# MoFHeka/MeepoEmbedding

Hardware: AMD Instinct MI355X
Metric: key-lookups/sec (higher is better)
Workload: dtype int64 keys / fp32 rows (copy)

## Files before the change

include/meepo_embedding.h:

```cpp
#ifndef MEEPO_EMBEDDING_H
#define MEEPO_EMBEDDING_H
#include <stddef.h>
#include <stdint.h>

#ifdef __cplusplus
extern "C" {
#endif

#define MEE_ABI_VERSION 2

#define MEE_EMPTY_KEY     INT64_MIN
#define MEE_RECLAIMED_KEY (INT64_MIN + 1)
#define MEE_BUCKET_WIDTH  16

enum { MEE_OK = 0, MEE_ERR_INVALID_ARG = -1, MEE_ERR_OUT_OF_MEMORY = -2, MEE_ERR_HIP = -3,
       MEE_ERR_NO_DEVICE = -4, MEE_ERR_BATCH_TOO_LARGE = -5, MEE_ERR_UNSUPPORTED = -6,
       MEE_ERR_RCCL = -7  };

enum { MEE_OPT_NONE = 0, MEE_OPT_ADAGRAD = 1, MEE_OPT_ADAM = 2 };
enum { MEE_INIT_CONSTANT = 0, MEE_INIT_UNIFORM = 1 };
enum { MEE_STATUS_TABLE_FULL = 1u, MEE_STATUS_RESERVED_KEY = 2u, MEE_STATUS_STALE_HANDLE = 4u, MEE_STATUS_INTERNAL = 8u };
enum { MEE_MEM_HBM = 0, MEE_MEM_HOST_PINNED = 1 };
enum { MEE_FLAG_TRACK_HITS = 1u, MEE_FLAG_ADMISSION = 2u };

// ... 175 lines not shown
                    void* stream);

int mee_bag_runs(mee_router* r, const int64_t* d_perm, const uint64_t* d_counts, size_t n, const uint64_t* d_bag_offsets, size_t n_bags,
                 uint32_t* d_run_bag, uint32_t* d_run_len, uint64_t* d_run_counts, void* stream);
int mee_run_offsets(mee_router* r, const uint32_t* d_run_len, size_t n_runs, uint64_t* d_offsets, uint32_t* d_run_of_key, size_t n_keys,
                    void* stream);
int mee_combine_bag_runs(mee_router* r, const float* d_partials, const uint32_t* d_run_bag, const uint64_t* d_run_counts, size_t n_runs,
                         const uint64_t* d_bag_offsets, size_t n_bags, uint32_t dim, int mode, void* d_out, uint32_t out_dtype, void* stream);

int mee_segment_counts(mee_router* r, const int64_t* d_perm, const uint64_t* d_counts, size_t n, const uint64_t* d_offsets, size_t n_tables,
                       uint64_t* d_cell_counts, void* stream);
int mee_regroup(mee_router* r, const int64_t* d_recv_keys, const uint64_t* d_recv_cells, size_t n_recv, size_t n_tables, int64_t* d_keys_out,
                int64_t* d_order_out, uint64_t* d_offsets_out, void* stream);

int mee_p2p_create(int32_t device, uint32_t n_shards, uint32_t rank, uint64_t slots_per_peer, uint64_t max_batch, uint32_t dim,
                   int with_payload, mee_p2p** out);
int mee_p2p_destroy(mee_p2p* c);
#define MEE_P2P_BUFFERS 6
int mee_p2p_export(mee_p2p* c, void* handles );
int mee_p2p_connect(mee_p2p* c, const void* all_handles );
int mee_p2p_buffers(mee_p2p* c, float** d_out, uint8_t** d_found);
int mee_p2p_push(mee_p2p* c, mee_router* r, const int64_t* d_send_keys, const int64_t* d_perm, const uint64_t* d_counts, size_t n,
                 void* stream);
int mee_p2p_find(mee_p2p* c, const mee_table* t, void* stream);
int mee_p2p_push_rows(mee_p2p* c, mee_router* r, const int64_t* d_send_keys, const int64_t* d_perm, const uint64_t* d_counts,
                      const float* d_rows, size_t n, void* stream);
int mee_p2p_inbox(mee_p2p* c, int64_t** d_keys, float** d_rows, uint64_t* n_slots);
int mee_p2p_barrier(mee_p2p* c, void* stream);
int mee_p2p_status(mee_p2p* c, uint32_t* bits_out, void* stream);


#define MEE_COMM_ID_BYTES 128
int mee_comm_unique_id(void* id_out );
int mee_comm_create(const void* id, uint32_t n_ranks, uint32_t rank, int32_t device, void** comm_out);
int mee_comm_destroy(void* comm);
int mee_comm_aborted(void* comm);
int mee_sharded_create(mee_table* local, void* nccl_comm, uint64_t max_batch ,
                       double pad_slack, mee_sharded** out);
enum { MEE_SHARDED_DEDUP = 1u };
typedef struct mee_sharded_options {
    uint32_t struct_size;
    uint32_t flags;
    uint64_t max_batch;
    double   pad_slack;
    mee_table* cold;
    uint64_t hot_key_limit;
} mee_sharded_options;
int mee_sharded_create_ex(mee_table* local, void* nccl_comm, const mee_sharded_options* options, mee_sharded** out);
int mee_sharded_destroy(mee_sharded* s);
int mee_sharded_info(const mee_sharded* s, uint32_t* n_shards, uint32_t* rank, uint64_t* segment_capacity );
int mee_sharded_find(mee_sharded* s, const int64_t* d_keys, size_t n, float* d_out, uint8_t* d_found , void* stream);
int mee_sharded_find_or_insert(mee_sharded* s, const int64_t* d_keys, size_t n, float* d_out, uint8_t* d_found, void* stream);
// ... 18 lines not shown
```

include/meepo_embedding.hpp:

```cpp
#pragma once
#include <cstdint>
#include <stdexcept>
#include <string>
#include <utility>

#include "meepo_embedding.h"

namespace meepo {

class Error : public std::runtime_error {
public:
    Error(int code, const std::string& msg) : std::runtime_error("meepo error " + std::to_string(code) + ": " + msg), code_(code) {}
    int code() const noexcept { return code_; }
private:
    int code_;
};

inline void check(int rc) {
    if (rc != MEE_OK) throw Error(rc, mee_last_error());
}

struct TableOptions {
    int32_t device = 0;
    uint64_t capacity = 0;
// ... 152 lines not shown
    Router(Router&& o) noexcept : r_(std::exchange(o.r_, nullptr)) {}
    Router(const Router&) = delete;
    Router& operator=(const Router&) = delete;
    mee_router* handle() const noexcept { return r_; }
    void partition(const int64_t* d_keys, size_t n, int64_t* d_send_keys, uint64_t* d_counts, int64_t* d_perm, void* stream = nullptr) { check(mee_partition(r_, d_keys, n, d_send_keys, d_counts, d_perm, stream)); }
    void partition_padded(const int64_t* d_keys, size_t n, int64_t* d_send_keys, uint64_t* d_counts, int64_t* d_perm, void* stream = nullptr) { check(mee_partition_padded(r_, d_keys, n, d_send_keys, d_counts, d_perm, stream)); }
    static void scatter_rows(const void* d_rows, const int64_t* d_perm, size_t n, size_t row_bytes, void* d_out, void* stream = nullptr) { check(mee_scatter_rows(d_rows, d_perm, n, row_bytes, d_out, stream)); }
    static void gather_rows(const void* d_rows, const int64_t* d_perm, size_t n, size_t row_bytes, void* d_out, void* stream = nullptr) { check(mee_gather_rows(d_rows, d_perm, n, row_bytes, d_out, stream)); }
private:
    mee_router* r_ = nullptr;
};

class PeerExchange {
public:
    PeerExchange(int32_t device, uint32_t n_shards, uint32_t rank, uint64_t slots_per_peer, uint64_t max_batch, uint32_t dim, bool with_payload = false) {
        check(mee_p2p_create(device, n_shards, rank, slots_per_peer, max_batch, dim, with_payload ? 1 : 0, &c_));
    }
    ~PeerExchange() { if (c_) mee_p2p_destroy(c_); }
    PeerExchange(const PeerExchange&) = delete;
    PeerExchange& operator=(const PeerExchange&) = delete;
    void export_handles(void* handles_6x64) { check(mee_p2p_export(c_, handles_6x64)); }
    void connect(const void* all_handles_rank_major) { check(mee_p2p_connect(c_, all_handles_rank_major)); }
    void push(Router& r, const int64_t* d_send_keys, const int64_t* d_perm, const uint64_t* d_counts, size_t n, void* stream = nullptr) { check(mee_p2p_push(c_, r.handle(), d_send_keys, d_perm, d_counts, n, stream)); }
    void find(const Table& t, void* stream = nullptr) { check(mee_p2p_find(c_, t.handle(), stream)); }
    void barrier(void* stream = nullptr) { check(mee_p2p_barrier(c_, stream)); }
    void push_rows(Router& r, const int64_t* d_send_keys, const int64_t* d_perm, const uint64_t* d_counts, const float* d_rows, size_t n, void* stream = nullptr) {
        check(mee_p2p_push_rows(c_, r.handle(), d_send_keys, d_perm, d_counts, d_rows, n, stream));
    }
    int64_t* inbox_keys() const { int64_t* k = nullptr; check(mee_p2p_inbox(c_, &k, nullptr, nullptr)); return k; }
    float* inbox_rows() const { float* r = nullptr; check(mee_p2p_inbox(c_, nullptr, &r, nullptr)); return r; }
    uint64_t inbox_slots() const { uint64_t n = 0; check(mee_p2p_inbox(c_, nullptr, nullptr, &n)); return n; }
    float* rows() const { float* o = nullptr; check(mee_p2p_buffers(c_, &o, nullptr)); return o; }
    uint8_t* found() const { uint8_t* f = nullptr; check(mee_p2p_buffers(c_, nullptr, &f)); return f; }
    uint32_t status(void* stream = nullptr) { uint32_t b = 0; check(mee_p2p_status(c_, &b, stream)); return b; }
private:
    mee_p2p* c_ = nullptr;
};

class Communicator {
public:
    static void unique_id(void* id_128_bytes) { check(mee_comm_unique_id(id_128_bytes)); }
    Communicator(const void* id_128_bytes, uint32_t n_ranks, uint32_t rank, int32_t device) { check(mee_comm_create(id_128_bytes, n_ranks, rank, device, &c_)); }
    ~Communicator() { if (c_) mee_comm_destroy(c_); }
    Communicator(const Communicator&) = delete;
    Communicator& operator=(const Communicator&) = delete;
    void* handle() const noexcept { return c_; }
private:
    void* c_ = nullptr;
};

class ShardedTable {
public:
    ShardedTable(Table& local, void* nccl_comm, uint64_t max_batch, double pad_slack = 0.0) { check(mee_sharded_create(local.handle(), nccl_comm, max_batch, pad_slack, &s_)); }
    ShardedTable(Table& local, void* nccl_comm, uint64_t max_batch, double pad_slack, Table* cold, uint32_t flags = 0, uint64_t hot_key_limit = 0) {
        mee_sharded_options o{};
        o.struct_size = sizeof o; o.flags = flags; o.max_batch = max_batch; o.pad_slack = pad_slack; o.cold = cold ? cold->handle() : nullptr; o.hot_key_limit = hot_key_limit;
        check(mee_sharded_create_ex(local.handle(), nccl_comm, &o, &s_));
// ... 23 lines not shown
```

meepoembedding_amd/_lib.py:

```python
from __future__ import annotations

import ctypes as C
import os

import torch

_HERE = os.path.dirname(os.path.abspath(__file__))
LIB_PATH = os.environ.get("MEE_LIB_PATH") or os.path.join(_HERE, "libmeepo_hip.so")

OK = 0
ERR_INVALID_ARG, ERR_OUT_OF_MEMORY, ERR_HIP, ERR_NO_DEVICE, ERR_BATCH_TOO_LARGE, ERR_UNSUPPORTED, ERR_RCCL = -1, -2, -3, -4, -5, -6, -7
OPT_NONE, OPT_ADAGRAD, OPT_ADAM = 0, 1, 2
INIT_CONSTANT, INIT_UNIFORM = 0, 1
STATUS_TABLE_FULL, STATUS_RESERVED_KEY, STATUS_STALE_HANDLE, STATUS_INTERNAL = 1, 2, 4, 8
FIND_DEFAULT, FIND_STREAM_STORES, FIND_CACHED_STORES, FIND_STREAM_ROWS, FIND_STREAM_BUCKETS = 0, 1, 2, 4, 8
HANDLE_SLOT_MASK = (1 << 40) - 1
MEM_HBM, MEM_HOST_PINNED = 0, 1
DTYPE_F32, DTYPE_BF16 = 0, 1
FLAG_TRACK_HITS, FLAG_ADMISSION = 1, 2
ABI_VERSION = 2
EMPTY_KEY = -(1 << 63)
RECLAIMED_KEY = EMPTY_KEY + 1
BUCKET_WIDTH = 16

# ... 108 lines not shown
    "mee_table_plane": (C.c_int, [_vp, _u32, C.POINTER(_vp), C.POINTER(_u64), C.POINTER(_u32)]),
    "mee_device_calibration": (C.c_int, [C.c_int32, C.POINTER(Calibration)]),
    "mee_probe_length": (C.c_int, [_vp, _vp, _sz, C.POINTER(_u64), _vp]),
    "mee_probe_histogram": (C.c_int, [_vp, _vp, _sz, C.POINTER(C.c_uint64), _vp]),
    "mee_apply_adagrad": (C.c_int, [_vp, _vp, _vp, _sz, _f32, _f32, _vp]),
    "mee_apply_adam": (C.c_int, [_vp, _vp, _vp, _sz, _f32, _f32, _f32, _f32, _u64, _vp]),
    "mee_apply_prepare": (C.c_int, [_vp, _vp, _sz, _vp]),
    "mee_apply_discard": (C.c_int, [_vp, _vp]),
    "mee_dedup_sum": (C.c_int, [_vp, _vp, _vp, _sz, _vp, _vp, _vp, _vp, C.c_int64, _vp]),
    "mee_hash_batch": (C.c_int, [_vp, _sz, _u64, _u32, _vp, _vp, _vp, _vp]),
    "mee_router_create": (C.c_int, [_i32, _u64, _u32, C.POINTER(_vp)]),
    "mee_router_destroy": (C.c_int, [_vp]),
    "mee_partition_padded": (C.c_int, [_vp, _vp, _sz, _vp, _vp, _vp, _vp]),
    "mee_partition": (C.c_int, [_vp, _vp, _sz, _vp, _vp, _vp, _vp]),
    "mee_p2p_create": (C.c_int, [_i32, _u32, _u32, _u64, _u64, _u32, C.c_int, C.POINTER(_vp)]),
    "mee_p2p_barrier": (C.c_int, [_vp, _vp]),
    "mee_p2p_push_rows": (C.c_int, [_vp, _vp, _vp, _vp, _vp, _vp, _sz, _vp]),
    "mee_p2p_inbox": (C.c_int, [_vp, C.POINTER(_vp), C.POINTER(_vp), C.POINTER(_u64)]),
    "mee_p2p_destroy": (C.c_int, [_vp]),
    "mee_p2p_export": (C.c_int, [_vp, _vp]),
    "mee_p2p_connect": (C.c_int, [_vp, _vp]),
    "mee_p2p_buffers": (C.c_int, [_vp, C.POINTER(_vp), C.POINTER(_vp)]),
    "mee_p2p_push": (C.c_int, [_vp, _vp, _vp, _vp, _vp, _sz, _vp]),
    "mee_p2p_find": (C.c_int, [_vp, _vp, _vp]),
    "mee_p2p_status": (C.c_int, [_vp, C.POINTER(_u32), _vp]),
    "mee_scatter_rows": (C.c_int, [_vp, _vp, _sz, _sz, _vp, _vp]),
    "mee_gather_rows": (C.c_int, [_vp, _vp, _sz, _sz, _vp, _vp]),
    "mee_bag_runs": (C.c_int, [_vp, _vp, _vp, _sz, _vp, _sz, _vp, _vp, _vp, _vp]),
    "mee_run_offsets": (C.c_int, [_vp, _vp, _sz, _vp, _vp, _sz, _vp]),
    "mee_combine_bag_runs": (C.c_int, [_vp, _vp, _vp, _vp, _sz, _vp, _sz, _u32, C.c_int, _vp, _u32, _vp]),
    "mee_segment_counts": (C.c_int, [_vp, _vp, _vp, _sz, _vp, _sz, _vp, _vp]),
    "mee_regroup": (C.c_int, [_vp, _vp, _vp, _sz, _sz, _vp, _vp, _vp, _vp]),
    "mee_comm_unique_id": (C.c_int, [_vp]),
    "mee_comm_create": (C.c_int, [_vp, _u32, _u32, _i32, C.POINTER(_vp)]),
    "mee_comm_destroy": (C.c_int, [_vp]),
    "mee_comm_aborted": (C.c_int, [_vp]),
    "mee_sharded_create": (C.c_int, [_vp, _vp, _u64, C.c_double, C.POINTER(_vp)]),
    "mee_sharded_create_ex": (C.c_int, [_vp, _vp, C.POINTER(ShardedOptions), C.POINTER(_vp)]),
    "mee_sharded_clear_status": (C.c_int, [_vp, _vp]),
    "mee_sharded_destroy": (C.c_int, [_vp]),
    "mee_sharded_info": (C.c_int, [_vp, C.POINTER(_u32), C.POINTER(_u32), C.POINTER(_u64)]),
    "mee_sharded_find": (C.c_int, [_vp, _vp, _sz, _vp, _vp, _vp]),
    "mee_sharded_find_or_insert": (C.c_int, [_vp, _vp, _sz, _vp, _vp, _vp]),
    "mee_sharded_find_as": (C.c_int, [_vp, _vp, _sz, _vp, _u32, _vp, _vp]),
    "mee_sharded_find_or_insert_as": (C.c_int, [_vp, _vp, _sz, _vp, _u32, _vp, _vp]),
    "mee_sharded_traffic": (C.c_int, [_vp, C.POINTER(_u64), C.POINTER(_u64)]),
# ... 45 lines not shown
```

meepoembedding_amd/csrc/meepo_router.hip:

```cpp
#include <hip/hip_runtime.h>

#include <cstdlib>
#include <cstring>
#include <new>

#include "meepo_device.h"
#include "meepo_host.h"

struct mee_router {
    int device;
    uint64_t max_batch;
    uint32_t n_shards;
    uint32_t max_blocks;
    uint32_t* blockcnt;
    uint64_t* base;
    uint64_t* run_base;
    uint64_t* run_sums;
};

struct mee_p2p {
    int device;
    uint32_t n_shards, rank, dim;
    uint64_t cap, max_batch;
    int64_t* inbox_keys;
    int32_t* inbox_dst;
    uint32_t* inbox_cnt;
    float* out;
    uint8_t* found;
    float* inbox_rows;
    uint32_t* status;
    void** d_tables;
    void* h_tables[6][64];
    bool connected;
};

namespace mee {

constexpr int kPartBlock = 1024;
constexpr int kMaxShards = 64;
constexpr uint32_t kNoOwner = 0xFFFFFFFFu;

template <class T>
__device__ __forceinline__ T wave_scan_inclusive(T v, int lane) {
#pragma unroll
    for (int d = 1; d < 64; d <<= 1) {
        const T t = __shfl_up(v, d);
        if (lane >= d) v += t;
    }
    return v;
}

template <bool RANK>
__device__ __forceinline__ uint32_t count_owners(uint32_t o, uint32_t g, uint32_t (&wcnt)[kPartBlock / 64][kMaxShards]) {
    const int lane = threadIdx.x & 63, w = threadIdx.x >> 6;
    uint32_t r = 0;
    for (uint32_t p = 0; p < g; ++p) {
        const uint64_t m = __ballot(o == p);
        if (RANK && o == p) r = (uint32_t)__popcll(m & ((1ull << lane) - 1));
        if (lane == 0) wcnt[w][p] = (uint32_t)__popcll(m);
    }
    __syncthreads();
    if (RANK && o != kNoOwner)
        for (int ww = 0; ww < w; ++ww) r += wcnt[ww][o];
    return r;
}
__device__ __forceinline__ void store_block_counts(const uint32_t (&wcnt)[kPartBlock / 64][kMaxShards], uint32_t g, uint32_t* blockcnt) {
    if (threadIdx.x < g) {
        uint32_t c = 0;
#pragma unroll
        for (int ww = 0; ww < kPartBlock / 64; ++ww) c += wcnt[ww][threadIdx.x];
        blockcnt[(uint64_t)blockIdx.x * g + threadIdx.x] = c;
    }
}

__global__ void hash_batch_kernel(const int64_t* __restrict__ keys, uint64_t n, uint64_t nb, uint32_t g, uint64_t* mix_out,
                                  uint64_t* bucket_out, uint32_t* owner_out) {
    for (uint64_t i = blockIdx.x * (uint64_t)blockDim.x + threadIdx.x; i < n; i += (uint64_t)gridDim.x * blockDim.x) {
        const int64_t k = keys[i];
        if (mix_out) mix_out[i] = mix64((uint64_t)k);
        if (bucket_out) bucket_out[i] = bucket_of(k, nb);
        if (owner_out) owner_out[i] = owner_of(k, g);
    }
}

template <bool SKIP_PAD>
__global__ __launch_bounds__(kPartBlock) void part_count_kernel(const int64_t* __restrict__ keys, uint32_t n, uint32_t g,
                                                                uint32_t* blockcnt) {
    __shared__ uint32_t wcnt[kPartBlock / 64][kMaxShards];
    const uint32_t i = blockIdx.x * kPartBlock + threadIdx.x;
    const int64_t key = i < n ? keys[i] : kEmpty;
    const bool inb = i < n && !(SKIP_PAD && key == kEmpty);
    count_owners<false>(inb ? owner_of(key, g) : kNoOwner, g, wcnt);
    store_block_counts(wcnt, g, blockcnt);
}

__global__ __launch_bounds__(1024) void part_scan_kernel(uint32_t* blockcnt, uint32_t n_blocks, uint32_t g, uint64_t* base,
                                                         uint64_t* counts_out) {
    __shared__ uint64_t total[kMaxShards];
    const int lane = threadIdx.x & 63, w = threadIdx.x >> 6, nw = blockDim.x >> 6;
    for (uint32_t p = w; p < g; p += nw) {
        uint32_t run = 0;
        for (uint32_t b0 = 0; b0 < n_blocks; b0 += 64) {
            const uint32_t b = b0 + lane;
            const uint32_t c = b < n_blocks ? blockcnt[(uint64_t)b * g + p] : 0;
            const uint32_t incl = wave_scan_inclusive(c, lane);
            if (b < n_blocks) blockcnt[(uint64_t)b * g + p] = run + incl - c;
            run += __shfl(incl, 63);
        }
        if (lane == 0) total[p] = run;
    }
    __syncthreads();
    if (threadIdx.x == 0) {
        uint64_t acc = 0;
        for (uint32_t p = 0; p < g; ++p) {
            base[p] = acc;
            counts_out[p] = total[p];
            acc += total[p];
        }
    }
}

template <bool SKIP_PAD>
__global__ __launch_bounds__(kPartBlock) void part_scatter_kernel(const int64_t* __restrict__ keys, uint32_t n, uint32_t g,
                                                                  const uint32_t* __restrict__ blockoff,
                                                                  const uint64_t* __restrict__ base, int64_t* send_keys,
                                                                  int64_t* perm) {
    __shared__ uint32_t wcnt[kPartBlock / 64][kMaxShards];
    const uint32_t i = blockIdx.x * kPartBlock + threadIdx.x;
    const int64_t key = i < n ? keys[i] : kEmpty;
    const bool inb = i < n && !(SKIP_PAD && key == kEmpty);
    const uint32_t o = inb ? owner_of(key, g) : kNoOwner;
    const uint32_t r = count_owners<true>(o, g, wcnt);
    if (inb) {
        const uint64_t dst = base[o] + blockoff[(uint64_t)blockIdx.x * g + o] + r;
        send_keys[dst] = key;
        perm[dst] = (int64_t)i;
    }
}

template <typename T, bool SCATTER>
__global__ void permute_rows_kernel(const T* __restrict__ rows, const int64_t* __restrict__ perm, uint64_t n, uint32_t epr,
                                    T* __restrict__ out) {
    const uint64_t total = n * epr;
    for (uint64_t idx = blockIdx.x * (uint64_t)blockDim.x + threadIdx.x; idx < total; idx += (uint64_t)gridDim.x * blockDim.x) {
        const uint64_t q = idx / epr;
        const uint32_t e = (uint32_t)(idx - q * epr);
        const uint64_t p = (uint64_t)perm[q];
        if (SCATTER) out[p * epr + e] = rows[idx];
        else out[idx] = rows[p * epr + e];
    }
}

template <bool SCATTER>
static int permute_rows(const void* d_rows, const int64_t* d_perm, size_t n, size_t row_bytes, void* d_out, void* stream,
                        const char* name) {
    if (n && (!d_rows || !d_perm || !d_out)) return fail(MEE_ERR_INVALID_ARG, "%s: null argument", name);
    if (n == 0 || row_bytes == 0) return MEE_OK;
// ... 45 lines not shown
    const uint32_t q = blockIdx.x * kPartBlock + threadIdx.x;
    const bool inb = q < s_end[g - 1];
    uint32_t seg = 0;
    while (seg + 1 < g && s_end[seg] <= q) ++seg;
    const uint32_t seg_begin = seg ? s_end[seg - 1] : 0;
    const uint32_t bag = inb ? last_not_above(off, n_bags, (uint64_t)perm[q]) : 0;
    s_bag[threadIdx.x] = bag;
    __syncthreads();
    uint32_t prev = 0;
    if (inb && q > seg_begin) prev = threadIdx.x ? s_bag[threadIdx.x - 1] : last_not_above(off, n_bags, (uint64_t)perm[q - 1]);
    RunPos r;
    r.head = inb && (q == seg_begin || bag != prev);
    r.seg = r.head ? seg : kNoOwner;
    r.bag = bag;
    r.seg_end = s_end[seg];
    return r;
}

__global__ __launch_bounds__(kPartBlock) void run_count_kernel(const int64_t* __restrict__ perm, const uint64_t* __restrict__ counts, uint32_t g, uint32_t n,
                                                              const uint64_t* __restrict__ off, uint32_t n_bags, uint32_t* blockcnt) {
    __shared__ uint32_t s_end[kMaxShards], s_bag[kPartBlock], wcnt[kPartBlock / 64][kMaxShards];
    const RunPos r = run_position(perm, counts, g, n, off, n_bags, s_end, s_bag);
    count_owners<false>(r.seg, g, wcnt);
    store_block_counts(wcnt, g, blockcnt);
}

__global__ __launch_bounds__(kPartBlock) void run_scatter_kernel(const int64_t* __restrict__ perm, const uint64_t* __restrict__ counts, uint32_t g, uint32_t n,
                                                                const uint64_t* __restrict__ off, uint32_t n_bags, const uint32_t* __restrict__ blockoff,
                                                                const uint64_t* __restrict__ run_base, uint32_t* __restrict__ run_bag,
                                                                uint32_t* __restrict__ run_len) {
    __shared__ uint32_t s_end[kMaxShards], s_bag[kPartBlock], wcnt[kPartBlock / 64][kMaxShards];
    const RunPos r = run_position(perm, counts, g, n, off, n_bags, s_end, s_bag);
    const uint32_t rank = count_owners<true>(r.seg, g, wcnt);
    if (r.head) {
        const uint64_t dst = run_base[r.seg] + blockoff[(uint64_t)blockIdx.x * g + r.seg] + rank;
        const uint32_t q = blockIdx.x * kPartBlock + threadIdx.x;
        const uint64_t bag_end = off[r.bag + 1];
        uint32_t lo = q + 1, hi = r.seg_end;
        while (lo < hi) {
            const uint32_t mid = lo + (hi - lo) / 2;
            if ((uint64_t)perm[mid] < bag_end) lo = mid + 1; else hi = mid;
        }
        run_bag[dst] = r.bag;
        run_len[dst] = lo - q;
    }
}

// ... 217 lines not shown
        if (two && q0 + 1 >= dst_off[c + 1]) {
            const uint32_t c1 = lds_last_not_above(dst_off, n_cells, q0 + 1);
            const uint32_t j1 = c1 / g, s1 = c1 - j1 * g;
            src1 = (uint64_t)src_off[s1 * n_tables + j1] + (q0 + 1 - dst_off[c1]);
        }
        const bool ok0 = src < n_recv, ok1 = two && src1 < n_recv;
        longlong2 k = make_longlong2(kEmpty, kEmpty);
        if (ok0 && ok1 && src1 == src + 1 && (src & 1) == 0) k = *reinterpret_cast<const longlong2*>(recv_keys + src);
        else {
            if (ok0) k.x = recv_keys[src];
            if (ok1) k.y = recv_keys[src1];
        }
        if (ok0 && ok1) {
            *reinterpret_cast<longlong2*>(keys_out + q0) = k;
            *reinterpret_cast<longlong2*>(order_out + q0) = make_longlong2((long long)src, (long long)src1);
        } else {
            if (ok0) { keys_out[q0] = k.x; order_out[q0] = (int64_t)src; }
            if (ok1) { keys_out[q0 + 1] = k.y; order_out[q0 + 1] = (int64_t)src1; }
        }
    }
}

constexpr int kP2PBuffers = 6;
struct P2PPeers {
    int64_t** keys; int32_t** dst; uint32_t** cnt; float** out; uint8_t** found; float** rows;
};

__global__ __launch_bounds__(256) void p2p_push_kernel(const int64_t* __restrict__ send_keys, const int64_t* __restrict__ perm,
                                                       const uint64_t* __restrict__ counts, const uint64_t* __restrict__ base,
                                                       P2PPeers peers, uint32_t me, uint64_t cap, uint32_t* status, int pad) {
    const uint32_t p = blockIdx.y;
    const uint64_t cnt = counts[p];
    const uint64_t take = cnt < cap ? cnt : cap;
    int64_t* __restrict__ dk = peers.keys[p] + (uint64_t)me * cap;
    int32_t* __restrict__ dd = peers.dst[p] + (uint64_t)me * cap;
    const uint64_t b0 = base[p];
    for (uint64_t j = blockIdx.x * (uint64_t)blockDim.x + threadIdx.x; j < take; j += (uint64_t)gridDim.x * blockDim.x) {
        dk[j] = send_keys[b0 + j];
        dd[j] = (int32_t)perm[b0 + j];
    }
    if (pad)
        for (uint64_t j = take + blockIdx.x * (uint64_t)blockDim.x + threadIdx.x; j < cap; j += (uint64_t)gridDim.x * blockDim.x) dk[j] = kEmpty;
    if (blockIdx.x == 0 && threadIdx.x == 0) {
        peers.cnt[p][me] = (uint32_t)take;
        if (cnt > cap) atomicOr(status, 1u);
    }
}

__global__ __launch_bounds__(64) void p2p_barrier_kernel(P2PPeers peers, uint32_t me, uint32_t n_shards, uint32_t* status,
// ... 97 lines not shown
}

using namespace mee;

extern "C" {

int mee_hash_batch(const int64_t* d_keys, size_t n, uint64_t n_buckets, uint32_t n_shards, uint64_t* d_mix_out,
                   uint64_t* d_bucket_out, uint32_t* d_owner_out, void* stream) {
    MEE_RANGE("mee_hash_batch");
    if (n && !d_keys) return fail(MEE_ERR_INVALID_ARG, "mee_hash_batch: null keys");
    if (n == 0) return MEE_OK;
    hash_batch_kernel<<<grid_for(n, 256, 1u << 14), 256, 0, (hipStream_t)stream>>>(d_keys, n, n_buckets, n_shards, d_mix_out,
                                                                                 d_bucket_out, d_owner_out);
    MEE_HIP(hipGetLastError());
    return MEE_OK;
}

int mee_router_destroy(mee_router* r) {
    MEE_RANGE("mee_router_destroy");
    if (!r) return MEE_OK;
    DeviceGuard g(r->device);
    if (r->blockcnt) (void)hipFree(r->blockcnt);
    if (r->base) (void)hipFree(r->base);
    if (r->run_base) (void)hipFree(r->run_base);
    if (r->run_sums) (void)hipFree(r->run_sums);
    delete r;
    return MEE_OK;
}

int mee_router_create(int32_t device, uint64_t max_batch, uint32_t n_shards, mee_router** out) {
    MEE_RANGE("mee_router_create");
    if (!out) return fail(MEE_ERR_INVALID_ARG, "mee_router_create: null out");
    *out = nullptr;
    if (n_shards == 0 || n_shards > (uint32_t)kMaxShards || max_batch == 0 || max_batch > (1ull << 30))
        return fail(MEE_ERR_INVALID_ARG, "mee_router_create: n_shards must be 1..%d and max_batch 1..2^30", kMaxShards);
    int ndev = 0;
    if (hipGetDeviceCount(&ndev) != hipSuccess || ndev <= 0)
        return fail(MEE_ERR_NO_DEVICE, "mee_router_create: no HIP device visible (this backend has no CPU fallback)");
    if (device < 0 || device >= ndev) return fail(MEE_ERR_INVALID_ARG, "mee_router_create: device %d out of range", device);
    DeviceGuard g(device);
    mee_router* r = new (std::nothrow) mee_router();
    if (!r) return fail(MEE_ERR_OUT_OF_MEMORY, "host allocation failed");
    r->device = device; r->max_batch = max_batch; r->n_shards = n_shards;
    r->max_blocks = (uint32_t)((max_batch + kPartBlock - 1) / kPartBlock);
    r->blockcnt = nullptr; r->base = nullptr; r->run_base = nullptr; r->run_sums = nullptr;
    if (hipMalloc((void**)&r->blockcnt, (size_t)r->max_blocks * n_shards * 4) != hipSuccess ||
        hipMalloc((void**)&r->base, n_shards * 8) != hipSuccess || hipMalloc((void**)&r->run_base, n_shards * 8) != hipSuccess ||
        hipMalloc((void**)&r->run_sums, ((size_t)r->max_blocks * n_shards + 1) * 8) != hipSuccess) {
        mee_router_destroy(r);
        return fail(MEE_ERR_OUT_OF_MEMORY, "mee_router_create: hipMalloc failed");
    }
    *out = r;
    return MEE_OK;
}

static int partition_common(mee_router* r, const int64_t* d_keys, size_t n, int64_t* d_send_keys, uint64_t* d_counts, int64_t* d_perm,
                            void* stream, bool skip_pad, const char* name) {
    if (!r || !d_counts || (n && (!d_keys || !d_send_keys || !d_perm))) return fail(MEE_ERR_INVALID_ARG, "%s: null argument", name);
    if (n > r->max_batch) return fail(MEE_ERR_BATCH_TOO_LARGE, "%s: n=%zu exceeds max_batch=%llu", name, n, (unsigned long long)r->max_batch);
    DeviceGuard g(r->device);
    hipStream_t st = (hipStream_t)stream;
    const uint32_t nblk = (uint32_t)((n + kPartBlock - 1) / kPartBlock);
    if (nblk) with_flag(skip_pad, [&](auto sp) { part_count_kernel<sp><<<nblk, kPartBlock, 0, st>>>(d_keys, (uint32_t)n, r->n_shards, r->blockcnt); });
    part_scan_kernel<<<1, 1024, 0, st>>>(r->blockcnt, nblk, r->n_shards, r->base, d_counts);
    if (nblk) with_flag(skip_pad, [&](auto sp) { part_scatter_kernel<sp><<<nblk, kPartBlock, 0, st>>>(d_keys, (uint32_t)n, r->n_shards, r->blockcnt, r->base, d_send_keys, d_perm); });
    MEE_HIP(hipGetLastError());
    return MEE_OK;
}
int mee_partition(mee_router* r, const int64_t* d_keys, size_t n, int64_t* d_send_keys, uint64_t* d_counts, int64_t* d_perm,
                  void* stream) {
    MEE_RANGE("mee_partition");
    return partition_common(r, d_keys, n, d_send_keys, d_counts, d_perm, stream, false, "mee_partition");
}
int mee_partition_padded(mee_router* r, const int64_t* d_keys, size_t n, int64_t* d_send_keys, uint64_t* d_counts, int64_t* d_perm,
                         void* stream) {
    MEE_RANGE("mee_partition_padded");
    return partition_common(r, d_keys, n, d_send_keys, d_counts, d_perm, stream, true, "mee_partition_padded");
}

int mee_bag_runs(mee_router* r, const int64_t* d_perm, const uint64_t* d_counts, size_t n, const uint64_t* d_bag_offsets, size_t n_bags,
                 uint32_t* d_run_bag, uint32_t* d_run_len, uint64_t* d_run_counts, void* stream) {
    MEE_RANGE("mee_bag_runs");
    if (!r || !d_counts || !d_bag_offsets || !d_run_counts || (n && (!d_perm || !d_run_bag || !d_run_len)))
        return fail(MEE_ERR_INVALID_ARG, "mee_bag_runs: null argument");
    if (n > r->max_batch) return fail(MEE_ERR_BATCH_TOO_LARGE, "mee_bag_runs: n=%zu exceeds max_batch=%llu", n, (unsigned long long)r->max_batch);
    if (n_bags > 0xFFFFFFFFull || (n && n_bags == 0)) return fail(MEE_ERR_INVALID_ARG, "mee_bag_runs: n_bags must be in [1, 2^32) when there are positions (the bags partition them)");
    DeviceGuard g(r->device);
    hipStream_t st = (hipStream_t)stream;
// ... 185 lines not shown
    P2PPeers pp;
    pp.keys = (int64_t**)(c->d_tables + 0 * (size_t)c->n_shards);
    pp.dst = (int32_t**)(c->d_tables + 1 * (size_t)c->n_shards);
    pp.cnt = (uint32_t**)(c->d_tables + 2 * (size_t)c->n_shards);
    pp.out = (float**)(c->d_tables + 3 * (size_t)c->n_shards);
    pp.found = (uint8_t**)(c->d_tables + 4 * (size_t)c->n_shards);
    pp.rows = (float**)(c->d_tables + 5 * (size_t)c->n_shards);
    return pp;
}

int mee_p2p_push(mee_p2p* c, mee_router* r, const int64_t* d_send_keys, const int64_t* d_perm, const uint64_t* d_counts, size_t n,
                 void* stream) {
    MEE_RANGE("mee_p2p_push");
    if (!c || !r || !d_counts || (n && (!d_send_keys || !d_perm))) return fail(MEE_ERR_INVALID_ARG, "mee_p2p_push: null argument");
    if (!c->connected) return fail(MEE_ERR_INVALID_ARG, "mee_p2p_push: not connected");
    if (r->n_shards != c->n_shards || n > c->max_batch) return fail(MEE_ERR_INVALID_ARG, "mee_p2p_push: router/batch mismatch");
    DeviceGuard g(c->device);
    const dim3 grid(grid_for(n / c->n_shards + 256, 256, 1024), c->n_shards);
    p2p_push_kernel<<<grid, 256, 0, (hipStream_t)stream>>>(d_send_keys, d_perm, d_counts, r->base, p2p_peers(c), c->rank, c->cap, c->status, 0);
    MEE_HIP(hipGetLastError());
    return MEE_OK;
}

int mee_p2p_push_rows(mee_p2p* c, mee_router* r, const int64_t* d_send_keys, const int64_t* d_perm, const uint64_t* d_counts,
                      const float* d_rows, size_t n, void* stream) {
    MEE_RANGE("mee_p2p_push_rows");
    if (!c || !r || !d_counts || (n && (!d_send_keys || !d_perm))) return fail(MEE_ERR_INVALID_ARG, "mee_p2p_push_rows: null argument");
    if (!c->connected || !c->inbox_rows) return fail(MEE_ERR_INVALID_ARG, "mee_p2p_push_rows: context not connected or created without payload");
    if (r->n_shards != c->n_shards || n > c->max_batch) return fail(MEE_ERR_INVALID_ARG, "mee_p2p_push_rows: router/batch mismatch");
    DeviceGuard g(c->device);
    hipStream_t st = (hipStream_t)stream;
    const dim3 gk(grid_for(c->cap, 256, 1024), c->n_shards);
    p2p_push_kernel<<<gk, 256, 0, st>>>(d_send_keys, d_perm, d_counts, r->base, p2p_peers(c), c->rank, c->cap, c->status, 1);
    if (d_rows) {
        const dim3 gr(grid_for(n / c->n_shards + 64, 16, 4096), c->n_shards);
        p2p_push_rows_kernel<<<gr, 256, 0, st>>>((const float4*)d_rows, d_perm, d_counts, r->base, p2p_peers(c), c->rank, c->cap, c->dim / 4);
    }
    MEE_HIP(hipGetLastError());
    return MEE_OK;
}

int mee_p2p_inbox(mee_p2p* c, int64_t** d_keys, float** d_rows, uint64_t* n_slots) {
    if (!c) return fail(MEE_ERR_INVALID_ARG, "mee_p2p_inbox: null argument");
    if (d_keys) *d_keys = c->inbox_keys;
    if (d_rows) *d_rows = c->inbox_rows;
    if (n_slots) *n_slots = (uint64_t)c->n_shards * c->cap;
// ... 16 lines not shown
    MEE_HIP(hipGetLastError());
    return MEE_OK;
}

int mee_p2p_barrier(mee_p2p* c, void* stream) {
    MEE_RANGE("mee_p2p_barrier");
    if (!c) return fail(MEE_ERR_INVALID_ARG, "mee_p2p_barrier: null argument");
    if (!c->connected) return fail(MEE_ERR_INVALID_ARG, "mee_p2p_barrier: not connected");
    DeviceGuard g(c->device);
    p2p_barrier_kernel<<<1, 64, 0, (hipStream_t)stream>>>(p2p_peers(c), c->rank, c->n_shards, c->status, 500000000ull);
    MEE_HIP(hipGetLastError());
    return MEE_OK;
}

int mee_p2p_status(mee_p2p* c, uint32_t* bits_out, void* stream) {
    MEE_RANGE("mee_p2p_status");
    if (!c || !bits_out) return fail(MEE_ERR_INVALID_ARG, "mee_p2p_status: null argument");
    DeviceGuard g(c->device);
    MEE_HIP(hipMemcpyAsync(bits_out, c->status, 4, hipMemcpyDeviceToHost, (hipStream_t)stream));
    MEE_HIP(hipStreamSynchronize((hipStream_t)stream));
    return MEE_OK;
}

int mee_scatter_rows(const void* d_rows, const int64_t* d_perm, size_t n, size_t row_bytes, void* d_out, void* stream) {
    MEE_RANGE("mee_scatter_rows");
    return permute_rows<true>(d_rows, d_perm, n, row_bytes, d_out, stream, "mee_scatter_rows");
}
int mee_gather_rows(const void* d_rows, const int64_t* d_perm, size_t n, size_t row_bytes, void* d_out, void* stream) {
    MEE_RANGE("mee_gather_rows");
    return permute_rows<false>(d_rows, d_perm, n, row_bytes, d_out, stream, "mee_gather_rows");
}

}
```

meepoembedding_amd/p2p.py:

```python
from __future__ import annotations

import ctypes as C

import torch
import torch.distributed as dist

from . import _lib
from ._lib import check


class _Raw:

    def __init__(self, ptr: int, shape, typestr: str):
        self.__cuda_array_interface__ = {"shape": tuple(shape), "typestr": typestr, "data": (ptr, False), "version": 2}


class PeerShardedFind:
    def __init__(self, local, router, max_batch: int, group=None, slack: float = 1.25, payload: bool = False,
                 device_barrier: bool = True):
        self.local, self.router, self.group = local, router, group
        self.world, self.rank = dist.get_world_size(group), dist.get_rank(group)
        self.device, self.dim, self.max_batch = local.device, local.dim, max_batch
        if router.n_shards != self.world:
            raise ValueError("router shards != process group size")
# ... 53 lines not shown
            except Exception:
                pass
            _lib.lib().mee_p2p_destroy(self._h)
            self._h = None

    def _barrier(self) -> None:
        if self.device_barrier and self._h:
            check(_lib.lib().mee_p2p_barrier(self._h, torch.cuda.current_stream(self.device).cuda_stream))
        elif self._staged:
            torch.cuda.synchronize(self.device)
            dist.barrier(group=self.group)
        else:
            dist.all_reduce(self._tok, group=self.group)

    def find(self, keys: torch.Tensor, check_overflow: bool = True, dedup: bool = False):
        keys = keys.contiguous().view(-1)
        n = keys.numel()
        if n > self.max_batch:
            raise _lib.MeepoError(_lib.ERR_BATCH_TOO_LARGE, f"n={n} exceeds max_batch={self.max_batch}")
        L = _lib.lib()
        s = torch.cuda.current_stream(self.device).cuda_stream
        if dedup:
            uniq, inverse = self.local.dedup_keys(keys, miss_index=self.max_batch)
            send_keys, counts, perm = self.router.partition(uniq, skip_padding=True)
            check(L.mee_p2p_push(self._h, self.router._h, send_keys.data_ptr(), perm.data_ptr(), counts.data_ptr(), n, s))
            self._barrier()
            check(L.mee_p2p_find(self._h, self.local._h, s))
            self._barrier()
            if check_overflow:
                self.check()
            rows = self.router.gather_rows(self.out, inverse, n_out=n)
            found = self.router.gather_rows(self.found, inverse, n_out=n)
            return rows, found
        send_keys, counts, perm = self.router.partition(keys)
        check(L.mee_p2p_push(self._h, self.router._h, send_keys.data_ptr(), perm.data_ptr(), counts.data_ptr(), n, s))
        self._barrier()
        check(L.mee_p2p_find(self._h, self.local._h, s))
        self._barrier()
        if check_overflow:
            self.check()
        return self.out[:n], self.found[:n]

    def find_or_insert(self, keys: torch.Tensor, check_overflow: bool = True):
        if not self.payload:
            raise _lib.MeepoError(_lib.ERR_INVALID_ARG, "find_or_insert needs PeerShardedFind(..., payload=True)")
        keys = keys.contiguous().view(-1)
        n = keys.numel()
        if n > self.max_batch:
            raise _lib.MeepoError(_lib.ERR_BATCH_TOO_LARGE, f"n={n} exceeds max_batch={self.max_batch}")
        L = _lib.lib()
        s = torch.cuda.current_stream(self.device).cuda_stream
        send_keys, counts, perm = self.router.partition(keys)
        check(L.mee_p2p_push_rows(self._h, self.router._h, send_keys.data_ptr(), perm.data_ptr(), counts.data_ptr(), None, n, s))
        self._barrier()
        self.local.find_or_insert(self.inbox_keys, out=self.inbox_rows, found=self._ensure_found)
        check(L.mee_p2p_find(self._h, self.local._h, s))
        self._barrier()
        if check_overflow:
# ... 32 lines not shown
        self._deliver(keys, values)
        self.local.assign(self.inbox_keys, self.inbox_rows)
        self._done(check_overflow)

    def apply_adagrad(self, keys: torch.Tensor, grads: torch.Tensor, lr: float, eps: float = 1e-10, check_overflow: bool = True, dedup: bool = False) -> None:
        self._deliver(keys, grads, aggregate=dedup)
        self.local.apply_adagrad(self.inbox_keys, self.inbox_rows, lr, eps)
        self._done(check_overflow)

    def apply_adam(self, keys: torch.Tensor, grads: torch.Tensor, lr: float, beta1: float = 0.9, beta2: float = 0.999,
                   eps: float = 1e-8, step: int = 1, check_overflow: bool = True, dedup: bool = False) -> None:
        self._deliver(keys, grads)
        self.local.apply_adam(self.inbox_keys, self.inbox_rows, lr, beta1, beta2, eps, step)
        self._done(check_overflow)

    def check(self) -> None:
        bits = C.c_uint32()
        check(_lib.lib().mee_p2p_status(self._h, C.byref(bits), torch.cuda.current_stream(self.device).cuda_stream))
        if bits.value & 2:
            raise _lib.MeepoError(_lib.ERR_HIP, "peer barrier timed out: a rank did not arrive within 5 s")
        if bits.value & 1:
            raise _lib.MeepoError(_lib.ERR_BATCH_TOO_LARGE, "peer inbox overflow: a rank sent more than slots_per_peer keys to one owner")


PeerShardedTable = PeerShardedFind
```

Baseline: 7.795 billion.

## Fuse key partitioning with peer push and drop scan kernel for small batches

Adds a partition_push entry point whose scatter kernel writes keys and destination indices straight into peer inboxes, skipping the intermediate send_keys/perm buffers and the separate p2p push kernel. For batches up to a block-count threshold, the count kernel stores counts owner-major and each scatter block computes its own offsets from all block counts, which removes the single-block scan kernel launch. The Python find path now uses the fused call. The cost is redundant per-block reduction work over all block counts, and peer-memory writes that are scattered rather than contiguous.

After: 7.771 billion. Within noise of the previous version (-0.3%).

```diff
diff --git a/include/meepo_embedding.h b/include/meepo_embedding.h
--- a/include/meepo_embedding.h
+++ b/include/meepo_embedding.h
@@ -221,12 +221,14 @@
 int mee_p2p_buffers(mee_p2p* c, float** d_out, uint8_t** d_found);
 int mee_p2p_push(mee_p2p* c, mee_router* r, const int64_t* d_send_keys, const int64_t* d_perm, const uint64_t* d_counts, size_t n,
                  void* stream);
+int mee_p2p_partition_push(mee_p2p* c, mee_router* r, const int64_t* d_keys, size_t n, int skip_padding, void* stream);
 int mee_p2p_find(mee_p2p* c, const mee_table* t, void* stream);
 int mee_p2p_push_rows(mee_p2p* c, mee_router* r, const int64_t* d_send_keys, const int64_t* d_perm, const uint64_t* d_counts,
                       const float* d_rows, size_t n, void* stream);
 int mee_p2p_inbox(mee_p2p* c, int64_t** d_keys, float** d_rows, uint64_t* n_slots);
 int mee_p2p_barrier(mee_p2p* c, void* stream);
 int mee_p2p_status(mee_p2p* c, uint32_t* bits_out, void* stream);
+int mee_p2p_clear_status(mee_p2p* c, void* stream);
 
 
 #define MEE_COMM_ID_BYTES 128
diff --git a/include/meepo_embedding.hpp b/include/meepo_embedding.hpp
--- a/include/meepo_embedding.hpp
+++ b/include/meepo_embedding.hpp
@@ -198,6 +198,7 @@
     void export_handles(void* handles_6x64) { check(mee_p2p_export(c_, handles_6x64)); }
     void connect(const void* all_handles_rank_major) { check(mee_p2p_connect(c_, all_handles_rank_major)); }
     void push(Router& r, const int64_t* d_send_keys, const int64_t* d_perm, const uint64_t* d_counts, size_t n, void* stream = nullptr) { check(mee_p2p_push(c_, r.handle(), d_send_keys, d_perm, d_counts, n, stream)); }
+    void partition_push(Router& r, const int64_t* d_keys, size_t n, bool skip_padding = false, void* stream = nullptr) { check(mee_p2p_partition_push(c_, r.handle(), d_keys, n, skip_padding ? 1 : 0, stream)); }
     void find(const Table& t, void* stream = nullptr) { check(mee_p2p_find(c_, t.handle(), stream)); }
     void barrier(void* stream = nullptr) { check(mee_p2p_barrier(c_, stream)); }
     void push_rows(Router& r, const int64_t* d_send_keys, const int64_t* d_perm, const uint64_t* d_counts, const float* d_rows, size_t n, void* stream = nullptr) {
@@ -209,6 +210,7 @@
     float* rows() const { float* o = nullptr; check(mee_p2p_buffers(c_, &o, nullptr)); return o; }
     uint8_t* found() const { uint8_t* f = nullptr; check(mee_p2p_buffers(c_, nullptr, &f)); return f; }
     uint32_t status(void* stream = nullptr) { uint32_t b = 0; check(mee_p2p_status(c_, &b, stream)); return b; }
+    void clear_status(void* stream = nullptr) { check(mee_p2p_clear_status(c_, stream)); }
 private:
     mee_p2p* c_ = nullptr;
 };
diff --git a/meepoembedding_amd/_lib.py b/meepoembedding_amd/_lib.py
--- a/meepoembedding_amd/_lib.py
+++ b/meepoembedding_amd/_lib.py
@@ -154,6 +154,8 @@
     "mee_p2p_connect": (C.c_int, [_vp, _vp]),
     "mee_p2p_buffers": (C.c_int, [_vp, C.POINTER(_vp), C.POINTER(_vp)]),
     "mee_p2p_push": (C.c_int, [_vp, _vp, _vp, _vp, _vp, _sz, _vp]),
+    "mee_p2p_partition_push": (C.c_int, [_vp, _vp, _vp, _sz, C.c_int, _vp]),
+    "mee_p2p_clear_status": (C.c_int, [_vp, _vp]),
     "mee_p2p_find": (C.c_int, [_vp, _vp, _vp]),
     "mee_p2p_status": (C.c_int, [_vp, C.POINTER(_u32), _vp]),
     "mee_scatter_rows": (C.c_int, [_vp, _vp, _sz, _sz, _vp, _vp]),
diff --git a/meepoembedding_amd/csrc/meepo_router.hip b/meepoembedding_amd/csrc/meepo_router.hip
--- a/meepoembedding_amd/csrc/meepo_router.hip
+++ b/meepoembedding_amd/csrc/meepo_router.hip
@@ -14,6 +14,7 @@
     uint32_t max_blocks;
     uint32_t* blockcnt;
     uint64_t* base;
+    uint64_t* totals;
     uint64_t* run_base;
     uint64_t* run_sums;
 };
@@ -39,6 +40,7 @@
 constexpr int kPartBlock = 1024;
 constexpr int kMaxShards = 64;
 constexpr uint32_t kNoOwner = 0xFFFFFFFFu;
+constexpr uint32_t kPartDirectBlocks = 2048;
 
 template <class T>
 __device__ __forceinline__ T wave_scan_inclusive(T v, int lane) {
@@ -64,13 +66,48 @@
         for (int ww = 0; ww < w; ++ww) r += wcnt[ww][o];
     return r;
 }
+template <bool BY_OWNER>
 __device__ __forceinline__ void store_block_counts(const uint32_t (&wcnt)[kPartBlock / 64][kMaxShards], uint32_t g, uint32_t* blockcnt) {
     if (threadIdx.x < g) {
         uint32_t c = 0;
 #pragma unroll
         for (int ww = 0; ww < kPartBlock / 64; ++ww) c += wcnt[ww][threadIdx.x];
-        blockcnt[(uint64_t)blockIdx.x * g + threadIdx.x] = c;
-    }
+        blockcnt[BY_OWNER ? (uint64_t)threadIdx.x * gridDim.x + blockIdx.x : (uint64_t)blockIdx.x * g + threadIdx.x] = c;
+    }
+}
+
+struct PartOffsets {
+    uint32_t off[kMaxShards], total[kMaxShards], base[kMaxShards];
+    uint32_t red[2][kPartBlock / 64][kMaxShards];
+};
+__device__ __forceinline__ void block_offsets(const uint32_t* __restrict__ cnt, uint32_t g, PartOffsets& s) {
+    const int lane = threadIdx.x & 63, w = threadIdx.x >> 6;
+    const uint32_t nblk = gridDim.x;
+    for (uint32_t p = 0; p < g; ++p) {
+        uint32_t before = 0, all = 0;
+        for (uint32_t b = threadIdx.x; b < nblk; b += kPartBlock) {
+            const uint32_t c = cnt[(uint64_t)p * nblk + b];
+            all += c;
+            before += b < blockIdx.x ? c : 0u;
+        }
+#pragma unroll
+        for (int d = 32; d >= 1; d >>= 1) {
+            before += __shfl_xor(before, d);
+            all += __shfl_xor(all, d);
+        }
+        if (lane == 0) { s.red[0][w][p] = before; s.red[1][w][p] = all; }
+    }
+    __syncthreads();
+    if (w == 0) {
+        uint32_t before = 0, all = 0;
+        if ((uint32_t)lane < g) {
+#pragma unroll
+            for (int ww = 0; ww < kPartBlock / 64; ++ww) { before += s.red[0][ww][lane]; all += s.red[1][ww][lane]; }
+        }
+        const uint32_t incl = wave_scan_inclusive(all, lane);
+        s.off[lane] = before; s.total[lane] = all; s.base[lane] = incl - all;
+    }
+    __syncthreads();
 }
 
 __global__ void hash_batch_kernel(const int64_t* __restrict__ keys, uint64_t n, uint64_t nb, uint32_t g, uint64_t* mix_out,
@@ -83,7 +120,7 @@
     }
 }
 
-template <bool SKIP_PAD>
+template <bool SKIP_PAD, bool BY_OWNER>
 __global__ __launch_bounds__(kPartBlock) void part_count_kernel(const int64_t* __restrict__ keys, uint32_t n, uint32_t g,
                                                                 uint32_t* blockcnt) {
     __shared__ uint32_t wcnt[kPartBlock / 64][kMaxShards];
@@ -91,7 +128,7 @@
     const int64_t key = i < n ? keys[i] : kEmpty;
     const bool inb = i < n && !(SKIP_PAD && key == kEmpty);
     count_owners<false>(inb ? owner_of(key, g) : kNoOwner, g, wcnt);
-    store_block_counts(wcnt, g, blockcnt);
+    store_block_counts<BY_OWNER>(wcnt, g, blockcnt);
 }
 
 __global__ __launch_bounds__(1024) void part_scan_kernel(uint32_t* blockcnt, uint32_t n_blocks, uint32_t g, uint64_t* base,
@@ -120,19 +157,54 @@
     }
 }
 
-template <bool SKIP_PAD>
-__global__ __launch_bounds__(kPartBlock) void part_scatter_kernel(const int64_t* __restrict__ keys, uint32_t n, uint32_t g,
-                                                                  const uint32_t* __restrict__ blockoff,
-                                                                  const uint64_t* __restrict__ base, int64_t* send_keys,
-                                                                  int64_t* perm) {
+struct P2PPeers {
+    int64_t** keys; int32_t** dst; uint32_t** cnt; float** out; uint8_t** found; float** rows;
+};
+struct PushSink { P2PPeers peers; uint32_t me; uint64_t cap; uint32_t* status; };
+
+template <bool SKIP_PAD, bool SCANNED, bool PUSH>
+__global__ __launch_bounds__(kPartBlock) void part_scatter_kernel(const int64_t* __restrict__ keys, uint32_t n, uint32_t g, const uint32_t* __restrict__ blockcnt,
+                                                                  uint64_t* base, uint64_t* counts, int64_t* send_keys, int64_t* perm, PushSink sink) {
     __shared__ uint32_t wcnt[kPartBlock / 64][kMaxShards];
+    __shared__ PartOffsets s;
+    __shared__ int64_t* s_keys[PUSH ? kMaxShards : 1];
+    __shared__ int32_t* s_dst[PUSH ? kMaxShards : 1];
+    if constexpr (SCANNED) {
+        if (threadIdx.x < g) {
+            s.off[threadIdx.x] = blockcnt[(uint64_t)blockIdx.x * g + threadIdx.x];
+            s.base[threadIdx.x] = (uint32_t)base[threadIdx.x];
+            s.total[threadIdx.x] = (uint32_t)counts[threadIdx.x];
+        }
+    } else {
+        block_offsets(blockcnt, g, s);
+        if (blockIdx.x == 0 && threadIdx.x < g) { base[threadIdx.x] = s.base[threadIdx.x]; counts[threadIdx.x] = s.total[threadIdx.x]; }
+    }
+    if constexpr (PUSH) {
+        if (threadIdx.x < g) {
+            s_keys[threadIdx.x] = sink.peers.keys[threadIdx.x] + (uint64_t)sink.me * sink.cap;
+            s_dst[threadIdx.x] = sink.peers.dst[threadIdx.x] + (uint64_t)sink.me * sink.cap;
+        }
+    }
     const uint32_t i = blockIdx.x * kPartBlock + threadIdx.x;
     const int64_t key = i < n ? keys[i] : kEmpty;
     const bool inb = i < n && !(SKIP_PAD && key == kEmpty);
     const uint32_t o = inb ? owner_of(key, g) : kNoOwner;
     const uint32_t r = count_owners<true>(o, g, wcnt);
-    if (inb) {
-        const uint64_t dst = base[o] + blockoff[(uint64_t)blockIdx.x * g + o] + r;
+    if constexpr (PUSH) {
+        if (blockIdx.x == 0 && threadIdx.x < g) {
+            const uint64_t cnt = s.total[threadIdx.x];
+            sink.peers.cnt[threadIdx.x][sink.me] = (uint32_t)(cnt < sink.cap ? cnt : sink.cap);
+            if (cnt > sink.cap) atomicOr(sink.status, 1u);
+        }
+        if (inb) {
+            const uint32_t j = s.off[o] + r;
+            if (j < sink.cap) {
+                s_keys[o][j] = key;
+                s_dst[o][j] = (int32_t)i;
+            }
+        }
+    } else if (inb) {
+        const uint64_t dst = (uint64_t)s.base[o] + s.off[o] + r;
         send_keys[dst] = key;
         perm[dst] = (int64_t)i;
     }
@@ -224,7 +296,7 @@
     __shared__ uint32_t s_end[kMaxShards], s_bag[kPartBlock], wcnt[kPartBlock / 64][kMaxShards];
     const RunPos r = run_position(perm, counts, g, n, off, n_bags, s_end, s_bag);
     count_owners<false>(r.seg, g, wcnt);
-    store_block_counts(wcnt, g, blockcnt);
+    store_block_counts<false>(wcnt, g, blockcnt);
 }
 
 __global__ __launch_bounds__(kPartBlock) void run_scatter_kernel(const int64_t* __restrict__ perm, const uint64_t* __restrict__ counts, uint32_t g, uint32_t n,
@@ -488,9 +560,6 @@
 }
 
 constexpr int kP2PBuffers = 6;
-struct P2PPeers {
-    int64_t** keys; int32_t** dst; uint32_t** cnt; float** out; uint8_t** found; float** rows;
-};
 
 __global__ __launch_bounds__(256) void p2p_push_kernel(const int64_t* __restrict__ send_keys, const int64_t* __restrict__ perm,
                                                        const uint64_t* __restrict__ counts, const uint64_t* __restrict__ base,
@@ -634,6 +703,7 @@
     DeviceGuard g(r->device);
     if (r->blockcnt) (void)hipFree(r->blockcnt);
     if (r->base) (void)hipFree(r->base);
+    if (r->totals) (void)hipFree(r->totals);
     if (r->run_base) (void)hipFree(r->run_base);
     if (r->run_sums) (void)hipFree(r->run_sums);
     delete r;
@@ -655,15 +725,27 @@
     if (!r) return fail(MEE_ERR_OUT_OF_MEMORY, "host allocation failed");
     r->device = device; r->max_batch = max_batch; r->n_shards = n_shards;
     r->max_blocks = (uint32_t)((max_batch + kPartBlock - 1) / kPartBlock);
-    r->blockcnt = nullptr; r->base = nullptr; r->run_base = nullptr; r->run_sums = nullptr;
+    r->blockcnt = nullptr; r->base = nullptr; r->totals = nullptr; r->run_base = nullptr; r->run_sums = nullptr;
     if (hipMalloc((void**)&r->blockcnt, (size_t)r->max_blocks * n_shards * 4) != hipSuccess ||
-        hipMalloc((void**)&r->base, n_shards * 8) != hipSuccess || hipMalloc((void**)&r->run_base, n_shards * 8) != hipSuccess ||
+        hipMalloc((void**)&r->base, n_shards * 8) != hipSuccess || hipMalloc((void**)&r->totals, n_shards * 8) != hipSuccess || hipMalloc((void**)&r->run_base, n_shards * 8) != hipSuccess ||
         hipMalloc((void**)&r->run_sums, ((size_t)r->max_blocks * n_shards + 1) * 8) != hipSuccess) {
         mee_router_destroy(r);
         return fail(MEE_ERR_OUT_OF_MEMORY, "mee_router_create: hipMalloc failed");
     }
     *out = r;
     return MEE_OK;
+}
+
+static void partition_launch(mee_router* r, const int64_t* d_keys, size_t n, int64_t* d_send_keys, uint64_t* d_counts, int64_t* d_perm, hipStream_t st,
+                             bool skip_pad, const PushSink* sink) {
+    const uint32_t nblk = n ? (uint32_t)((n + kPartBlock - 1) / kPartBlock) : 1u;
+    const uint32_t g = r->n_shards;
+    const PushSink sk = sink ? *sink : PushSink{};
+    with_flag(skip_pad, [&](auto sp) { with_flag(nblk > kPartDirectBlocks, [&](auto scanned) { with_flag(sink != nullptr, [&](auto push) {
+        part_count_kernel<sp, !scanned><<<nblk, kPartBlock, 0, st>>>(d_keys, (uint32_t)n, g, r->blockcnt);
+        if (scanned) part_scan_kernel<<<1, 1024, 0, st>>>(r->blockcnt, nblk, g, r->base, d_counts);
+        part_scatter_kernel<sp, scanned, push><<<nblk, kPartBlock, 0, st>>>(d_keys, (uint32_t)n, g, r->blockcnt, r->base, d_counts, d_send_keys, d_perm, sk);
+    }); }); });
 }
 
 static int partition_common(mee_router* r, const int64_t* d_keys, size_t n, int64_t* d_send_keys, uint64_t* d_counts, int64_t* d_perm,
@@ -671,11 +753,7 @@
     if (!r || !d_counts || (n && (!d_keys || !d_send_keys || !d_perm))) return fail(MEE_ERR_INVALID_ARG, "%s: null argument", name);
     if (n > r->max_batch) return fail(MEE_ERR_BATCH_TOO_LARGE, "%s: n=%zu exceeds max_batch=%llu", name, n, (unsigned long long)r->max_batch);
     DeviceGuard g(r->device);
-    hipStream_t st = (hipStream_t)stream;
-    const uint32_t nblk = (uint32_t)((n + kPartBlock - 1) / kPartBlock);
-    if (nblk) with_flag(skip_pad, [&](auto sp) { part_count_kernel<sp><<<nblk, kPartBlock, 0, st>>>(d_keys, (uint32_t)n, r->n_shards, r->blockcnt); });
-    part_scan_kernel<<<1, 1024, 0, st>>>(r->blockcnt, nblk, r->n_shards, r->base, d_counts);
-    if (nblk) with_flag(skip_pad, [&](auto sp) { part_scatter_kernel<sp><<<nblk, kPartBlock, 0, st>>>(d_keys, (uint32_t)n, r->n_shards, r->blockcnt, r->base, d_send_keys, d_perm); });
+    partition_launch(r, d_keys, n, d_send_keys, d_counts, d_perm, (hipStream_t)stream, skip_pad, nullptr);
     MEE_HIP(hipGetLastError());
     return MEE_OK;
 }
@@ -907,6 +985,19 @@
     return MEE_OK;
 }
 
+int mee_p2p_partition_push(mee_p2p* c, mee_router* r, const int64_t* d_keys, size_t n, int skip_padding, void* stream) {
+    MEE_RANGE("mee_p2p_partition_push");
+    if (!c || !r || (n && !d_keys)) return fail(MEE_ERR_INVALID_ARG, "mee_p2p_partition_push: null argument");
+    if (!c->connected) return fail(MEE_ERR_INVALID_ARG, "mee_p2p_partition_push: not connected");
+    if (r->n_shards != c->n_shards || r->device != c->device || n > c->max_batch) return fail(MEE_ERR_INVALID_ARG, "mee_p2p_partition_push: router/batch mismatch");
+    if (n > r->max_batch) return fail(MEE_ERR_BATCH_TOO_LARGE, "mee_p2p_partition_push: n=%zu exceeds the router's max_batch=%llu", n, (unsigned long long)r->max_batch);
+    DeviceGuard g(c->device);
+    const PushSink sink{p2p_peers(c), c->rank, c->cap, c->status};
+    partition_launch(r, d_keys, n, nullptr, r->totals, nullptr, (hipStream_t)stream, skip_padding != 0, &sink);
+    MEE_HIP(hipGetLastError());
+    return MEE_OK;
+}
+
 int mee_p2p_push_rows(mee_p2p* c, mee_router* r, const int64_t* d_send_keys, const int64_t* d_perm, const uint64_t* d_counts,
                       const float* d_rows, size_t n, void* stream) {
     MEE_RANGE("mee_p2p_push_rows");
@@ -969,6 +1060,14 @@
     return MEE_OK;
 }
 
+int mee_p2p_clear_status(mee_p2p* c, void* stream) {
+    MEE_RANGE("mee_p2p_clear_status");
+    if (!c) return fail(MEE_ERR_INVALID_ARG, "mee_p2p_clear_status: null argument");
+    DeviceGuard g(c->device);
+    MEE_HIP(hipMemsetAsync(c->status, 0, 4, (hipStream_t)stream));
+    return MEE_OK;
+}
+
 int mee_scatter_rows(const void* d_rows, const int64_t* d_perm, size_t n, size_t row_bytes, void* d_out, void* stream) {
     MEE_RANGE("mee_scatter_rows");
     return permute_rows<true>(d_rows, d_perm, n, row_bytes, d_out, stream, "mee_scatter_rows");
diff --git a/meepoembedding_amd/p2p.py b/meepoembedding_amd/p2p.py
--- a/meepoembedding_amd/p2p.py
+++ b/meepoembedding_amd/p2p.py
@@ -99,8 +99,7 @@
         s = torch.cuda.current_stream(self.device).cuda_stream
         if dedup:
             uniq, inverse = self.local.dedup_keys(keys, miss_index=self.max_batch)
-            send_keys, counts, perm = self.router.partition(uniq, skip_padding=True)
-            check(L.mee_p2p_push(self._h, self.router._h, send_keys.data_ptr(), perm.data_ptr(), counts.data_ptr(), n, s))
+            check(L.mee_p2p_partition_push(self._h, self.router._h, uniq.data_ptr(), n, 1, s))
             self._barrier()
             check(L.mee_p2p_find(self._h, self.local._h, s))
             self._barrier()
@@ -109,8 +108,7 @@
             rows = self.router.gather_rows(self.out, inverse, n_out=n)
             found = self.router.gather_rows(self.found, inverse, n_out=n)
             return rows, found
-        send_keys, counts, perm = self.router.partition(keys)
-        check(L.mee_p2p_push(self._h, self.router._h, send_keys.data_ptr(), perm.data_ptr(), counts.data_ptr(), n, s))
+        check(L.mee_p2p_partition_push(self._h, self.router._h, keys.data_ptr(), n, 0, s))
         self._barrier()
         check(L.mee_p2p_find(self._h, self.local._h, s))
         self._barrier()
@@ -189,5 +187,8 @@
         if bits.value & 1:
             raise _lib.MeepoError(_lib.ERR_BATCH_TOO_LARGE, "peer inbox overflow: a rank sent more than slots_per_peer keys to one owner")
 
+    def clear_status(self) -> None:
+        check(_lib.lib().mee_p2p_clear_status(self._h, torch.cuda.current_stream(self.device).cuda_stream))
+
 
 PeerShardedTable = PeerShardedFind
```
